# EmbersArc/SCpp

Hardware: AMD Instinct MI355X
Metric: converged SCvx trajectories/sec (RocketQuat, K=50) at 1/2/4/8 MI355X (higher is better)
Workload: dtype f64

## Files before the change

scpp_amd/csrc/discretize_kernel.h:

```cpp
#pragma once
#include "common.h"
#include <utility>

namespace scpp
{

template <class F, int... S>
__device__ inline void forEachStageImpl(F &&f, std::integer_sequence<int, S...>)
{
    (f(std::integral_constant<int, S>{}), ...);
}
template <class F>
__device__ inline void forEachStage(F &&f)
{
    forEachStageImpl(f, std::make_integer_sequence<int, RK_S>{});
}

#ifndef DISC_STEPS
#define DISC_STEPS 0
#endif
#ifndef DISC_MAX_STEP
#define DISC_MAX_STEP (12. / (14. * 5.))
#endif
constexpr int DISC_STEPS_MAX = 5;
#ifndef DISC_WAVES_PER_SIMD
#define DISC_WAVES_PER_SIMD 2
#endif

#ifndef DISC_STAGE_SCHEDULE
#define DISC_STAGE_SCHEDULE 1
#endif
#ifdef DISC_AD_JACOBIAN
#undef DISC_STAGE_SCHEDULE
#define DISC_STAGE_SCHEDULE 0
#endif
#ifndef DISC_LDS_GROUPS
#define DISC_LDS_GROUPS 1
#endif
#if defined(SCPP_HIP_EMU) || !DISC_LDS_GROUPS
#define DISC_READS_ISSUED()
#else
#define DISC_READS_ISSUED() __builtin_amdgcn_sched_barrier(0)
#endif
constexpr int rkNextStage(int s, bool skip)
{
    for (int r = s + 1; r < RK_S; r++)
        if (!skip || rkStageLive(r))
            return r;
    return RK_S;
}

template <class Model, bool FOH, bool VT>
struct DiscLayout
{
    static constexpr int NX = Model::NX, NU = Model::NU, NP = Model::NP;
    static constexpr int NJ = NX + NU;
    static constexpr int NCOLS = 1 + NX + NU + (FOH ? NU : 0) + (VT ? 1 : 0);
    static constexpr int NENT = NX * NCOLS;
    static constexpr int NG = WAVE / 16;
    static constexpr int EPL = (NCOLS + NG - 1) / NG;
    static constexpr int COL_S = 1, COL_PHI = 1 + (VT ? 1 : 0), COL_B = COL_PHI + NX, COL_C = COL_B + NU;
    static constexpr int NJP = (NJ + 1) & ~1;
};

template <class Model, bool FOH, bool VT>
struct DiscLds
{
    using L = DiscLayout<Model, FOH, VT>;
    __attribute__((aligned(16))) double Ys[32 * L::NX + 2];
#if DISC_STAGE_SCHEDULE
    __attribute__((aligned(16))) double Ys1[32 * L::NX + 2];
#endif
#ifdef DISC_AD_JACOBIAN
    __attribute__((aligned(16))) double Jm[L::NX * L::NJP];
    double fv[L::NX];
    double cst[L::NP + 2 * L::NU + 1];
#else
    double uh[DISC_STEPS_MAX * RK_S * (Model::JacobianRows::NUAUX + 1 + L::NU)];
    __attribute__((aligned(16))) double Wt[Model::JacobianTable::NW];
    double cst[L::NP + 2 * L::NU + Model::JacobianRows::NAUX + 1];
#endif
};

template <class Model, bool FOH, bool VT, bool SKIP = (RK_SKIP_DEAD != 0)>
__device__ __forceinline__ void discretizeSegment(int B, int K, const double *__restrict__ X, const double *__restrict__ U,
                                                  const double *__restrict__ sigma, const double *__restrict__ par, int par_stride,
                                                  const int *__restrict__ active, double *__restrict__ Aout, double *__restrict__ Bout,
                                                  double *__restrict__ Cout, double *__restrict__ Sout, double *__restrict__ Zout, int steps_opt,
                                                  const long inst, const int k, DiscLds<Model, FOH, VT> *lds)
{
    using L = DiscLayout<Model, FOH, VT>;
    constexpr int NX = L::NX, NU = L::NU, NP = L::NP, NJ = L::NJ, NJP = L::NJP, NCOLS = L::NCOLS, NG = L::NG, EPL = L::EPL;

    static_assert(NX <= 16 && NCOLS + NG <= 32 && NG == 4, "one 16-row tile of states, two 16-column tiles of V");
    auto &Ys = lds->Ys;
#ifndef DISC_AD_JACOBIAN
    constexpr int NAUX = Model::JacobianRows::NAUX;
    constexpr int NUAUX = Model::JacobianRows::NUAUX;
    constexpr int UHP = NUAUX + 1 + NU;
    auto &uh = lds->uh;
#define DISC_TABLE_ROWS 1
    using TB = typename Model::JacobianTable;
    auto &Wt = lds->Wt;
#else
    constexpr int NAUX = 0;
    auto &Jm = lds->Jm;
    auto &fv = lds->fv;
#endif
    auto &cst = lds->cst;

    const int lane = threadIdx.x;
    for (int i = lane; i < 32 * NX + 2; i += WAVE)
        Ys[i] = 0.;
    const int nseg = K - 1;
    if (inst >= B)
        return;
    if (active && active[inst] == 0)
        return;

    const double sg = sigma[inst];
    const double dt = VT ? 1. / double(K - 1) : sg / double(K - 1);
    const double tscale = VT ? sg : 1.;
    int nsteps = DISC_STEPS > 0 ? DISC_STEPS : steps_opt;
    if (nsteps <= 0)
    {
        const double seg_seconds = fabs(sg) / double(K - 1);
        nsteps = int(ceil(seg_seconds / DISC_MAX_STEP));
        nsteps = nsteps < 1 ? 1 : (nsteps > DISC_STEPS_MAX ? DISC_STEPS_MAX : nsteps);
    }
    nsteps = uniformInt(nsteps);
    double p[NP];
#pragma unroll
    for (int i = 0; i < NP; i++)
        p[i] = par[inst * par_stride + i];
    double u0[NU], u1[NU];
#pragma unroll
    for (int i = 0; i < NU; i++)
    {
        u0[i] = U[(inst * K + k) * NU + i];
        u1[i] = FOH ? U[(inst * K + k + 1) * NU + i] : u0[i];
    }

    if (lane == 0)
    {
#pragma unroll
        for (int i = 0; i < NP; i++)
            cst[i] = p[i];
#pragma unroll
        for (int i = 0; i < NU; i++)
        {
            cst[NP + i] = u0[i];
            cst[NP + NU + i] = u1[i];
        }
#ifndef DISC_AD_JACOBIAN
        double aux0[NAUX];
        Model::JacobianRows::prepare(p, aux0);
#pragma unroll
        for (int i = 0; i < NAUX; i++)
            cst[NP + 2 * NU + i] = aux0[i];
#endif
    }
#ifndef DISC_AD_JACOBIAN
    {
        const double hh = dt / double(nsteps);
        for (int e = lane; e < nsteps * RK_S; e += WAVE)
        {
            const double tse = double(e / RK_S) * hh + RK_C[e % RK_S] * hh;
            const double fre = FOH ? tse / dt : 0.;
            double ue[NU], ua[NUAUX];
#pragma unroll
            for (int i = 0; i < NU; i++)
                ue[i] = u0[i] + fre * (u1[i] - u0[i]);
            Model::JacobianRows::prepareInput(ue, p, ua);
#pragma unroll
            for (int i = 0; i < NUAUX; i++)
                uh[e * UHP + i] = ua[i];
            uh[e * UHP + NUAUX] = fre;
#pragma unroll
            for (int i = 0; i < NU; i++)
                uh[e * UHP + NUAUX + 1 + i] = ue[i];
        }
    }
#endif
#ifdef DISC_TABLE_ROWS
    for (int i = lane; i < TB::NW; i += WAVE)
        Wt[i] = (i == TB::W_ONE) ? 1. : 0.;
#endif
    WAVE_SYNC();
#ifdef DISC_TABLE_ROWS
    if (lane == 0)
    {
#pragma unroll
        for (int i = 0; i < NP; i++)
            Wt[TB::W_PAR + i] = p[i];
#pragma unroll
        for (int i = 0; i < NAUX; i++)
            Wt[TB::W_AUX + i] = cst[NP + 2 * NU + i];
    }
    double tcf[2][TB::MAXMON];
    unsigned tof[2][TB::MAXMON][2];
    int ttg[2];
#pragma unroll
    for (int ps = 0; ps < 2; ps++)
    {
        const int slot = ps * 64 + lane;
        ttg[ps] = TB::target(slot);
#pragma unroll
        for (int q = 0; q < TB::MAXMON; q++)
        {
            tcf[ps][q] = TB::coef(slot, q);
            tof[ps][q][0] = unsigned(TB::factor(slot, q, 0) * 8) | (unsigned(TB::factor(slot, q, 1) * 8) << 16);
            tof[ps][q][1] = unsigned(TB::factor(slot, q, 2) * 8) | (unsigned(TB::factor(slot, q, 3) * 8) << 16);
        }
    }
    WAVE_SYNC();
#endif
    const int row = lane & 15, g = lane >> 4;
    const bool lane_on = row < NX;
#ifndef SCPP_HIP_EMU
    __builtin_assume(g >= 0 && g < NG);
#endif
    const double x0r = lane_on ? X[(inst * K + k) * NX + row] : 0.;
    double y[EPL];
    bool eon[EPL];
#pragma unroll
    for (int m = 0; m < EPL; m++)
    {
        const int c = m * NG + g;
        eon[m] = lane_on && c < NCOLS;
        double v = 0.;
        if (c == 0)
            v = x0r;
        else if (c >= L::COL_PHI && c < L::COL_PHI + NX)
            v = (c - L::COL_PHI == row) ? 1. : 0.;
        y[m] = eon[m] ? v : 0.;
    }

    double kk[RK_S][EPL];
    const double h = dt / double(nsteps);
#ifdef DISC_PROFILE
    long long tA = 0, tB = 0, tC = 0;
    const long long tk0 = clock64();
#endif

    for (int step = 0; step < nsteps; step++)
    {
        const double t0 = double(step) * h;
        forEachStage([&](auto sc) {
            constexpr int s = decltype(sc)::value;
            if (SKIP && !rkStageLive(s))
                return;
#ifdef DISC_PROFILE
            const long long p0 = clock64();
#endif
            const double ts = t0 + RK_C[s] * h;
#pragma unroll
            for (int m = 0; m < EPL; m++)
            {
                double acc = 0.;
#pragma unroll
                for (int j = 0; j < s; j++)
                    if (RK_A[s][j] != 0.)
                        acc += RK_A[s][j] * kk[j][m];
                const double ys = y[m] + h * acc;
                if (eon[m])
                    Ys[(m * NG + g) * NX + row] = ys;
#ifdef DISC_TABLE_ROWS
                if (m == 0 && g == 0 && lane_on)
                    Wt[TB::W_X + row] = ys;
#endif
            }
            WAVE_SYNC();
#ifdef DISC_PROFILE
            const long long p1 = clock64();
            tA += p1 - p0;
#endif
#ifndef DISC_AD_JACOBIAN
            const double frac = FOH ? uh[(step * RK_S + s) * UHP + NUAUX] : 0.;
#else
            const double frac = FOH ? ts / dt : 0.;
#endif
            double jr[NJ];
            double fr;
#ifdef DISC_TABLE_ROWS
            double bsel[4];
            {
                const int e = step * RK_S + s;
                if (lane < NU)
                    Wt[TB::W_U + lane] = uh[e * UHP + NUAUX + 1 + lane];
                else if (lane < NU + NUAUX)
                    Wt[TB::W_UAUX + lane - NU] = uh[e * UHP + lane - NU];
                {
                    double hh[TB::NH];
                    TB::evalHoists(Ys, uh + e * UHP + NUAUX + 1, cst, cst + NP + 2 * NU, uh + e * UHP, hh);
                    if (lane == 0)
                    {
#pragma unroll
                        for (int i = 0; i < TB::NH; i++)
                            Wt[TB::W_H + i] = hh[i];
                    }
                }
                WAVE_SYNC();
                const char *wb = reinterpret_cast<const char *>(Wt);
#pragma unroll
                for (int ps = 0; ps < 2; ps++)
                {
                    double val = 0.;
#pragma unroll
                    for (int q = 0; q < (ps == 0 ? TB::MAXMON : TB::MAXMON_B); q++)
                    {
                        const double f0 = *reinterpret_cast<const double *>(wb + (tof[ps][q][0] & 0xFFFFu));
                        const double f1 = *reinterpret_cast<const double *>(wb + (tof[ps][q][0] >> 16));
                        const double f2 = *reinterpret_cast<const double *>(wb + (tof[ps][q][1] & 0xFFFFu));
                        const double f3 = *reinterpret_cast<const double *>(wb + (tof[ps][q][1] >> 16));
                        val += ((tcf[ps][q] * f0) * f1) * (f2 * f3);
                    }
                    if (ttg[ps] >= 0)
                        Wt[ttg[ps]] = val;
                    WAVE_SYNC();
                }
                const int rowc = lane_on ? row : 0;
#pragma unroll
                for (int t = 0; t < 4; t++)
                {
                    const double v = Wt[TB::W_J + rowc * NJ + (4 * t + g < NX ? 4 * t + g : 0)];
                    bsel[t] = (4 * t + g < NX) ? v : 0.;
                }
                fr = Wt[TB::W_F + rowc];
            }
#elif !defined(DISC_AD_JACOBIAN)
            {
                int zo = 0;
#ifndef SCPP_HIP_EMU
                asm volatile("" : "+v"(zo));
#endif
                const double *cv = cst + zo;
                double pl[NP], xs[NX], us[NU], ax[NAUX], ux[NUAUX];
#pragma unroll
                for (int i = 0; i < NUAUX; i++)
                    ux[i] = uh[(step * RK_S + s) * UHP + i];
#pragma unroll
                for (int i = 0; i < NP; i++)
                    pl[i] = cv[i];
#pragma unroll
                for (int i = 0; i < NAUX; i++)
                    ax[i] = cv[NP + 2 * NU + i];
#pragma unroll
                for (int i = 0; i < NX; i++)
                    xs[i] = Ys[i];
#pragma unroll
                for (int i = 0; i < NU; i++)
                {
                    const double a0 = cv[NP + i], a1 = cv[NP + NU + i];
                    us[i] = a0 + frac * (a1 - a0);
                }
                fr = Model::JacobianRows::row(row, xs, us, pl, ax, ux, jr);
            }
#else
            if (lane < NJ)
            {
                Dual1 xd[NX], ud[NU], fd[NX];
                int zo = 0;
#ifndef SCPP_HIP_EMU
                asm volatile("" : "+v"(zo));
#endif
                const double *cv = cst + zo;
                double pl[NP];
#pragma unroll
                for (int i = 0; i < NP; i++)
                    pl[i] = cv[i];
#pragma unroll
                for (int i = 0; i < NX; i++)
                    xd[i] = Dual1(Ys[i], (lane == i) ? 1. : 0.);
#pragma unroll
                for (int i = 0; i < NU; i++)
                {
                    const double a0 = cv[NP + i], a1 = cv[NP + NU + i];
                    ud[i] = Dual1(a0 + frac * (a1 - a0), (lane == NX + i) ? 1. : 0.);
                }
                Model::template systemFlowMap<Dual1>(xd, ud, pl, fd);
#pragma unroll
                for (int i = 0; i < NX; i++)
                    Jm[i * NJP + lane] = tscale * fd[i].d;
                if (lane == 0)
                {
#pragma unroll
                    for (int i = 0; i < NX; i++)
                        fv[i] = fd[i].v;
                }
            }
            WAVE_SYNC();
#pragma unroll
            for (int j = 0; j < NJ; j++)
                jr[j] = Jm[row * NJP + j];
            fr = fv[row];
#endif
#ifdef DISC_PROFILE
            const long long p2 = clock64();
            tB += p2 - p1;
#endif
            {
                const double alphaB = FOH ? (1. - frac) : 1.;
                d4_t acc0 = {0., 0., 0., 0.}, acc1 = {0., 0., 0., 0.};
#pragma unroll
                for (int t = 0; t < 4; t++)
                {
                    const int kx = g + 4 * t;
#ifdef DISC_TABLE_ROWS
                    double b = bsel[t];
#else
                    double b = (4 * t < NX) ? jr[4 * t < NX ? 4 * t : 0] : 0.;
#pragma unroll
                    for (int q = 1; q < 4; q++)
                        b = (g == q) ? ((4 * t + q < NX) ? jr[4 * t + q < NX ? 4 * t + q : 0] : 0.) : b;
#endif
#ifndef DISC_AD_JACOBIAN
                    b *= tscale;
#endif
                    acc0 = __builtin_amdgcn_mfma_f64_16x16x4f64(Ys[row * NX + kx], b, acc0, 0, 0, 0);
                    if (NCOLS > 16)
                        acc1 = __builtin_amdgcn_mfma_f64_16x16x4f64(Ys[(16 + row) * NX + kx], b, acc1, 0, 0, 0);
                }
#pragma unroll
                for (int m = 0; m < EPL; m++)
                {
                    const int c = m * NG + g;
                    const double acc = m < 4 ? acc0[m < 4 ? m : 0] : acc1[m >= 4 ? m - 4 : 0];
                    double d = acc;
                    const bool slotB = m * NG < L::COL_B + NU && m * NG + NG > L::COL_B;
                    const bool slotC = FOH && m * NG < L::COL_C + NU && m * NG + NG > L::COL_C;
                    if (slotB || slotC)
                    {
                        const bool isB = c >= L::COL_B && c < L::COL_B + NU;
                        const bool isC = FOH && c >= L::COL_C && c < L::COL_C + NU;
                        const int jj = isB ? c - L::COL_B : isC ? c - L::COL_C : 0;
                        const double w = isB ? alphaB : isC ? frac : 0.;
#ifdef DISC_TABLE_ROWS
                        const double jb = Wt[TB::W_J + (lane_on ? row : 0) * NJ + NX + jj];
#else
                        double jb = jr[NX];
#pragma unroll
                        for (int q = 1; q < NU; q++)
                            jb = (jj == q) ? jr[NX + q] : jb;
#endif
#ifndef DISC_AD_JACOBIAN
                        d += (w * tscale) * jb;
#else
                        d += w * jb;
#endif
                    }
                    if (VT && m * NG <= L::COL_S && m * NG + NG > L::COL_S)
                        d = (c == L::COL_S) ? d + fr : d;
                    if (m == 0)
                        d = (c == 0) ? tscale * fr : d;
                    kk[s][m] = d;
                }
            }
            WAVE_SYNC();
#ifdef DISC_PROFILE
            tC += clock64() - p2;
#endif
        });
#pragma unroll
        for (int m = 0; m < EPL; m++)
        {
            double acc = 0.;
#pragma unroll
            for (int s = 0; s < RK_S; s++)
                if (RK_B[s] != 0.)
                    acc += RK_B[s] * kk[s][m];
            y[m] += h * acc;
        }
    }

#ifdef DISC_PROFILE
    if (blockIdx.x == 4096 && lane == 0)
        printf("disc profile (cycles/segment): stage-value %lld  AD %lld  product %lld  total %lld\n", tA, tB, tC, (long long)(clock64() - tk0));
#endif
    const long seg = inst * nseg + k;
#pragma unroll
    for (int m = 0; m < EPL; m++)
    {
        const int c = m * NG + g;
        if (!eon[m])
            continue;
        Ys[c * NX + row] = y[m];
        if (c >= L::COL_PHI && c < L::COL_PHI + NX)
            Aout[seg * NX * NX + row * NX + (c - L::COL_PHI)] = y[m];
        else if (c >= L::COL_B && c < L::COL_B + NU)
            Bout[seg * NX * NU + row * NU + (c - L::COL_B)] = y[m];
        else if (FOH && c >= L::COL_C && c < L::COL_C + NU)
            Cout[seg * NX * NU + row * NU + (c - L::COL_C)] = y[m];
        else if (VT && c == L::COL_S)
            Sout[seg * NX + row] = y[m];
    }
    if (lane < NX)
        Ys[NCOLS * NX + lane] = x0r;
    WAVE_SYNC();
    if (lane < NX)
    {
        double z = Ys[lane];
#pragma unroll
        for (int j = 0; j < NX; j++)
            z -= Ys[(L::COL_PHI + j) * NX + lane] * Ys[NCOLS * NX + j];
#pragma unroll
        for (int j = 0; j < NU; j++)
        {
            z -= Ys[(L::COL_B + j) * NX + lane] * u0[j];
            if (FOH)
                z -= Ys[(L::COL_C + j) * NX + lane] * u1[j];
        }
        if (VT)
            z -= Ys[L::COL_S * NX + lane] * sg;
        Zout[seg * NX + lane] = z;
    }
}

#if DISC_STAGE_SCHEDULE
template <class Model>
struct DiscTableSlots
{
    using TB = typename Model::JacobianTable;
    double tcf[2][TB::MAXMON];
    unsigned tof[2][TB::MAXMON][2];
    int ttg[2];
};

template <class Model, bool FOH, bool VT>
__device__ __forceinline__ bool discretizeSetup(int B, const double *__restrict__ par, int par_stride, const int *__restrict__ active, const long inst,
                                                DiscLds<Model, FOH, VT> *lds, DiscTableSlots<Model> &ts)
{
    using L = DiscLayout<Model, FOH, VT>;
    using TB = typename Model::JacobianTable;
    constexpr int NX = L::NX, NU = L::NU, NP = L::NP, NAUX = Model::JacobianRows::NAUX;
    static_assert(NX <= 16 && L::NCOLS + L::NG <= 32 && L::NG == 4, "one 16-row tile of states, two 16-column tiles of V");
    const int lane = threadIdx.x;
    if (inst >= B)
        return false;
    if (active && active[inst] == 0)
        return false;
    for (int i = lane; i < 32 * NX + 2; i += WAVE)
    {
        lds->Ys[i] = 0.;
        lds->Ys1[i] = 0.;
    }
    for (int i = lane; i < TB::NW; i += WAVE)
        lds->Wt[i] = (i == TB::W_ONE) ? 1. : 0.;
    WAVE_SYNC();
    if (lane == 0)
    {
        double p[NP], aux0[NAUX];
#pragma unroll
        for (int i = 0; i < NP; i++)
            p[i] = par[inst * par_stride + i];
        Model::JacobianRows::prepare(p, aux0);
#pragma unroll
        for (int i = 0; i < NP; i++)
        {
            lds->cst[i] = p[i];
            lds->Wt[TB::W_PAR + i] = p[i];
        }
#pragma unroll
        for (int i = 0; i < NAUX; i++)
        {
            lds->cst[NP + 2 * NU + i] = aux0[i];
            lds->Wt[TB::W_AUX + i] = aux0[i];
        }
    }
#pragma unroll
    for (int ps = 0; ps < 2; ps++)
    {
        const int slot = ps * 64 + lane;
        ts.ttg[ps] = TB::target(slot);
#pragma unroll
        for (int q = 0; q < TB::MAXMON; q++)
        {
            ts.tcf[ps][q] = TB::coef(slot, q);
            ts.tof[ps][q][0] = unsigned(TB::factor(slot, q, 0) * 8) | (unsigned(TB::factor(slot, q, 1) * 8) << 16);
            ts.tof[ps][q][1] = unsigned(TB::factor(slot, q, 2) * 8) | (unsigned(TB::factor(slot, q, 3) * 8) << 16);
        }
    }
    WAVE_SYNC();
    return true;
}

template <class Model, bool FOH, bool VT, bool SKIP>
__device__ __forceinline__ void discretizeSegmentBody(int K, const double *__restrict__ X, const double *__restrict__ U, const double *__restrict__ sigma,
                                                      double *__restrict__ Aout, double *__restrict__ Bout, double *__restrict__ Cout,
                                                      double *__restrict__ Sout, double *__restrict__ Zout, int steps_opt, const long inst, const int k,
                                                      DiscLds<Model, FOH, VT> *lds, const DiscTableSlots<Model> &ts)
{
    using L = DiscLayout<Model, FOH, VT>;
    using TB = typename Model::JacobianTable;
    constexpr int NX = L::NX, NU = L::NU, NP = L::NP, NJ = L::NJ, NCOLS = L::NCOLS, NG = L::NG, EPL = L::EPL;
    constexpr int NAUX = Model::JacobianRows::NAUX, NUAUX = Model::JacobianRows::NUAUX, UHP = NUAUX + 1 + NU;
    constexpr int NLIVE = SKIP ? rkLiveBefore(RK_S) : RK_S;
    auto &Ys = lds->Ys;
    auto &uh = lds->uh;
    auto &Wt = lds->Wt;
    auto &cst = lds->cst;
    (void)NAUX;

    const int lane = threadIdx.x;
    const int nseg = K - 1;
    const double sg = sigma[inst];
    const double dt = VT ? 1. / double(K - 1) : sg / double(K - 1);
    const double tscale = VT ? sg : 1.;
    int nsteps = DISC_STEPS > 0 ? DISC_STEPS : steps_opt;
    if (nsteps <= 0)
    {
        const double seg_seconds = fabs(sg) / double(K - 1);
        nsteps = int(ceil(seg_seconds / DISC_MAX_STEP));
        nsteps = nsteps < 1 ? 1 : (nsteps > DISC_STEPS_MAX ? DISC_STEPS_MAX : nsteps);
    }
    nsteps = uniformInt(nsteps);
    const int row = lane & 15, g = lane >> 4;
    const bool lane_on = row < NX;
#ifndef SCPP_HIP_EMU
    __builtin_assume(g >= 0 && g < NG);
#endif
    double u0[NU], u1[NU];
#pragma unroll
    for (int i = 0; i < NU; i++)
    {
        u0[i] = U[(inst * K + k) * NU + i];
        u1[i] = FOH ? U[(inst * K + k + 1) * NU + i] : u0[i];
    }
#if DISC_LDS_GROUPS
    const double x0r = lane_on ? X[(inst * K + k) * NX + row] : 0.;
    DISC_READS_ISSUED();
#endif
    if (lane == 0)
    {
#pragma unroll
        for (int i = 0; i < NU; i++)
        {
            cst[NP + i] = u0[i];
            cst[NP + NU + i] = u1[i];
        }
    }
    {
        double p[NP];
#pragma unroll
        for (int i = 0; i < NP; i++)
            p[i] = cst[i];
        const double hh = dt / double(nsteps);
        for (int e = lane; e < nsteps * RK_S; e += WAVE)
        {
            const double tse = double(e / RK_S) * hh + RK_C[e % RK_S] * hh;
            const double fre = FOH ? tse / dt : 0.;
            double ue[NU], ua[NUAUX];
#pragma unroll
            for (int i = 0; i < NU; i++)
                ue[i] = u0[i] + fre * (u1[i] - u0[i]);
            Model::JacobianRows::prepareInput(ue, p, ua);
#pragma unroll
            for (int i = 0; i < NUAUX; i++)
                uh[e * UHP + i] = ua[i];
            uh[e * UHP + NUAUX] = fre;
#pragma unroll
            for (int i = 0; i < NU; i++)
                uh[e * UHP + NUAUX + 1 + i] = ue[i];
        }
    }
    WAVE_SYNC();

#if !DISC_LDS_GROUPS
    const double x0r = lane_on ? X[(inst * K + k) * NX + row] : 0.;
#endif
    double y[EPL];
    bool eon[EPL];
#pragma unroll
    for (int m = 0; m < EPL; m++)
    {
        const int c = m * NG + g;
        eon[m] = lane_on && c < NCOLS;
        double v = 0.;
        if (c == 0)
            v = x0r;
        else if (c >= L::COL_PHI && c < L::COL_PHI + NX)
            v = (c - L::COL_PHI == row) ? 1. : 0.;
        y[m] = eon[m] ? v : 0.;
    }

    double kk[RK_S][EPL];
    const double h = dt / double(nsteps);
#if DISC_LDS_GROUPS
    const bool ucp = lane < NU + NUAUX;
    const int usrc = lane < NU ? NUAUX + 1 + lane : (ucp ? lane - NU : 0);
    const int udst = lane < NU ? TB::W_U + lane : TB::W_UAUX + lane - NU;
    double uop_n = uh[usrc];
    double frac_n = FOH ? uh[NUAUX] : 0.;
#endif
    for (int step = 0; step < nsteps; step++)
    {
        forEachStage([&](auto sc) {
            constexpr int s = decltype(sc)::value;
            if (SKIP && !rkStageLive(s))
                return;
            constexpr int ord = SKIP ? rkLiveBefore(s) : s;
            const int buf = (NLIVE % 2 == 0) ? (ord & 1) : ((ord + step) & 1);
            double *Yb = buf ? lds->Ys1 : lds->Ys;
            const int e = step * RK_S + s;
            double ys0 = 0.;
#pragma unroll
            for (int m = 0; m < EPL; m++)
            {
                double acc = 0.;
#pragma unroll
                for (int j = 0; j < s; j++)
                    if (RK_A[s][j] != 0.)
                        acc += RK_A[s][j] * kk[j][m];
                const double ys = y[m] + h * acc;
                if (eon[m])
                    Yb[(m * NG + g) * NX + row] = ys;
                if (m == 0)
                {
                    ys0 = ys;
                    if (g == 0 && lane_on)
                        Wt[TB::W_X + row] = ys;
                }
            }
            {
                double xs[NX], hh[TB::NH];
#pragma unroll
                for (int i = 0; i < NX; i++)
                    xs[i] = readLane(ys0, i);
                TB::evalHoists(xs, uh + e * UHP + NUAUX + 1, cst, cst + NP + 2 * NU, uh + e * UHP, hh);
                if (lane == 0)
                {
#pragma unroll
                    for (int i = 0; i < TB::NH; i++)
                        Wt[TB::W_H + i] = hh[i];
                }
#if DISC_LDS_GROUPS
                if (ucp)
                    Wt[udst] = uop_n;
#else
                if (lane < NU)
                    Wt[TB::W_U + lane] = uh[e * UHP + NUAUX + 1 + lane];
                else if (lane < NU + NUAUX)
                    Wt[TB::W_UAUX + lane - NU] = uh[e * UHP + lane - NU];
#endif
            }
            WAVE_SYNC();
#if DISC_LDS_GROUPS
            const double frac = frac_n;
#else
            const double frac = FOH ? uh[e * UHP + NUAUX] : 0.;
#endif
            const char *wb = reinterpret_cast<const char *>(Wt);
#pragma unroll
            for (int ps = 0; ps < 2; ps++)
            {
                double val = 0.;
#if DISC_LDS_GROUPS
                double fc[TB::MAXMON][4];
#pragma unroll
                for (int q = 0; q < (ps == 0 ? TB::MAXMON : TB::MAXMON_B); q++)
                {
                    fc[q][0] = *reinterpret_cast<const double *>(wb + (ts.tof[ps][q][0] & 0xFFFFu));
                    fc[q][1] = *reinterpret_cast<const double *>(wb + (ts.tof[ps][q][0] >> 16));
                    fc[q][2] = *reinterpret_cast<const double *>(wb + (ts.tof[ps][q][1] & 0xFFFFu));
                    fc[q][3] = *reinterpret_cast<const double *>(wb + (ts.tof[ps][q][1] >> 16));
                }
                DISC_READS_ISSUED();
#pragma unroll
                for (int q = 0; q < (ps == 0 ? TB::MAXMON : TB::MAXMON_B); q++)
                    val += ((ts.tcf[ps][q] * fc[q][0]) * fc[q][1]) * (fc[q][2] * fc[q][3]);
#else
#pragma unroll
                for (int q = 0; q < (ps == 0 ? TB::MAXMON : TB::MAXMON_B); q++)
                {
                    const double f0 = *reinterpret_cast<const double *>(wb + (ts.tof[ps][q][0] & 0xFFFFu));
                    const double f1 = *reinterpret_cast<const double *>(wb + (ts.tof[ps][q][0] >> 16));
                    const double f2 = *reinterpret_cast<const double *>(wb + (ts.tof[ps][q][1] & 0xFFFFu));
                    const double f3 = *reinterpret_cast<const double *>(wb + (ts.tof[ps][q][1] >> 16));
                    val += ((ts.tcf[ps][q] * f0) * f1) * (f2 * f3);
                }
#endif
                if (ts.ttg[ps] >= 0)
                    Wt[ts.ttg[ps]] = val;
                WAVE_SYNC();
            }
            const int rowc = lane_on ? row : 0;
            double bsel[4];
#pragma unroll
            for (int t = 0; t < 4; t++)
            {
                const double v = Wt[TB::W_J + rowc * NJ + (4 * t + g < NX ? 4 * t + g : 0)];
#if DISC_LDS_GROUPS
                bsel[t] = v;
#else
                bsel[t] = (4 * t + g < NX) ? v : 0.;
#endif
            }
            const double fr = Wt[TB::W_F + rowc];
#if DISC_LDS_GROUPS
            auto forcingCol = [&](int m) {
                const int c = m * NG + g;
                const bool slotB = m * NG < L::COL_B + NU && m * NG + NG > L::COL_B;
                const bool slotC = FOH && m * NG < L::COL_C + NU && m * NG + NG > L::COL_C;
                if (!(slotB || slotC))
                    return -1;
                const bool isB = c >= L::COL_B && c < L::COL_B + NU;
                const bool isC = FOH && c >= L::COL_C && c < L::COL_C + NU;
                return isB ? c - L::COL_B : isC ? c - L::COL_C : 0;
            };
            double jbv[EPL], ya0[4], ya1[4];
#pragma unroll
            for (int m = 0; m < EPL; m++)
            {
                const int jj = forcingCol(m);
                jbv[m] = jj >= 0 ? Wt[TB::W_J + rowc * NJ + NX + jj] : 0.;
            }
#pragma unroll
            for (int t = 0; t < 4; t++)
            {
                ya0[t] = Yb[row * NX + g + 4 * t];
                ya1[t] = NCOLS > 16 ? Yb[(16 + row) * NX + g + 4 * t] : 0.;
            }
            {
                constexpr int sn = rkNextStage(s, SKIP);
                const int en = sn < RK_S ? step * RK_S + sn : (step + 1 < nsteps ? (step + 1) * RK_S : 0);
                uop_n = uh[en * UHP + usrc];
                frac_n = FOH ? uh[en * UHP + NUAUX] : 0.;
            }
            DISC_READS_ISSUED();
#pragma unroll
            for (int t = 0; t < 4; t++)
                bsel[t] = (4 * t + g < NX) ? bsel[t] : 0.;
#endif
            const double alphaB = FOH ? (1. - frac) : 1.;
            d4_t acc0 = {0., 0., 0., 0.}, acc1 = {0., 0., 0., 0.};
#pragma unroll
            for (int t = 0; t < 4; t++)
            {
                const int kx = g + 4 * t;
                const double b = bsel[t] * tscale;
#if DISC_LDS_GROUPS
                (void)kx;
                acc0 = __builtin_amdgcn_mfma_f64_16x16x4f64(ya0[t], b, acc0, 0, 0, 0);
                if (NCOLS > 16)
                    acc1 = __builtin_amdgcn_mfma_f64_16x16x4f64(ya1[t], b, acc1, 0, 0, 0);
#else
                acc0 = __builtin_amdgcn_mfma_f64_16x16x4f64(Yb[row * NX + kx], b, acc0, 0, 0, 0);
                if (NCOLS > 16)
                    acc1 = __builtin_amdgcn_mfma_f64_16x16x4f64(Yb[(16 + row) * NX + kx], b, acc1, 0, 0, 0);
#endif
            }
#pragma unroll
            for (int m = 0; m < EPL; m++)
            {
                const int c = m * NG + g;
                const double acc = m < 4 ? acc0[m < 4 ? m : 0] : acc1[m >= 4 ? m - 4 : 0];
                double d = acc;
                const bool slotB = m * NG < L::COL_B + NU && m * NG + NG > L::COL_B;
                const bool slotC = FOH && m * NG < L::COL_C + NU && m * NG + NG > L::COL_C;
                if (slotB || slotC)
                {
                    const bool isB = c >= L::COL_B && c < L::COL_B + NU;
                    const bool isC = FOH && c >= L::COL_C && c < L::COL_C + NU;
                    const int jj = isB ? c - L::COL_B : isC ? c - L::COL_C : 0;
                    const double w = isB ? alphaB : isC ? frac : 0.;
#if DISC_LDS_GROUPS
                    (void)jj;
                    const double jb = jbv[m];
#else
                    const double jb = Wt[TB::W_J + rowc * NJ + NX + jj];
#endif
                    d += (w * tscale) * jb;
                }
                if (VT && m * NG <= L::COL_S && m * NG + NG > L::COL_S)
                    d = (c == L::COL_S) ? d + fr : d;
                if (m == 0)
                    d = (c == 0) ? tscale * fr : d;
                kk[s][m] = d;
            }
        });
#pragma unroll
        for (int m = 0; m < EPL; m++)
        {
            double acc = 0.;
#pragma unroll
            for (int s = 0; s < RK_S; s++)
                if (RK_B[s] != 0.)
                    acc += RK_B[s] * kk[s][m];
            y[m] += h * acc;
        }
    }
    WAVE_SYNC();

    const long seg = inst * nseg + k;
#pragma unroll
    for (int m = 0; m < EPL; m++)
    {
        const int c = m * NG + g;
        if (!eon[m])
            continue;
        Ys[c * NX + row] = y[m];
        if (c >= L::COL_PHI && c < L::COL_PHI + NX)
            Aout[seg * NX * NX + row * NX + (c - L::COL_PHI)] = y[m];
        else if (c >= L::COL_B && c < L::COL_B + NU)
            Bout[seg * NX * NU + row * NU + (c - L::COL_B)] = y[m];
        else if (FOH && c >= L::COL_C && c < L::COL_C + NU)
            Cout[seg * NX * NU + row * NU + (c - L::COL_C)] = y[m];
        else if (VT && c == L::COL_S)
            Sout[seg * NX + row] = y[m];
    }
    if (lane < NX)
        Ys[NCOLS * NX + lane] = x0r;
    WAVE_SYNC();
    if (lane < NX)
    {
#if DISC_LDS_GROUPS
        double za[NX], zx[NX], zb[NU], zc[NU];
        double z = Ys[lane];
#pragma unroll
        for (int j = 0; j < NX; j++)
        {
            za[j] = Ys[(L::COL_PHI + j) * NX + lane];
            zx[j] = Ys[NCOLS * NX + j];
        }
#pragma unroll
        for (int j = 0; j < NU; j++)
        {
            zb[j] = Ys[(L::COL_B + j) * NX + lane];
            zc[j] = FOH ? Ys[(L::COL_C + j) * NX + lane] : 0.;
        }
        const double zs = VT ? Ys[L::COL_S * NX + lane] : 0.;
        DISC_READS_ISSUED();
#pragma unroll
        for (int j = 0; j < NX; j++)
            z -= za[j] * zx[j];
#pragma unroll
        for (int j = 0; j < NU; j++)
        {
            z -= zb[j] * u0[j];
            if (FOH)
                z -= zc[j] * u1[j];
        }
        if (VT)
            z -= zs * sg;
#else
        double z = Ys[lane];
#pragma unroll
        for (int j = 0; j < NX; j++)
            z -= Ys[(L::COL_PHI + j) * NX + lane] * Ys[NCOLS * NX + j];
#pragma unroll
        for (int j = 0; j < NU; j++)
        {
            z -= Ys[(L::COL_B + j) * NX + lane] * u0[j];
            if (FOH)
                z -= Ys[(L::COL_C + j) * NX + lane] * u1[j];
        }
        if (VT)
            z -= Ys[L::COL_S * NX + lane] * sg;
#endif
        Zout[seg * NX + lane] = z;
    }
    WAVE_SYNC();
    if (lane < NX)
        Ys[NCOLS * NX + lane] = 0.;
    WAVE_SYNC();
}
#endif

template <class Model, bool FOH, bool VT, int SCHED = DISC_STAGE_SCHEDULE, bool SKIP = (RK_SKIP_DEAD != 0)>
__device__ __forceinline__ void discretizeSegments(int B, int K, const double *__restrict__ X, const double *__restrict__ U,
                                                   const double *__restrict__ sigma, const double *__restrict__ par, int par_stride,
                                                   const int *__restrict__ active, double *__restrict__ Aout, double *__restrict__ Bout,
                                                   double *__restrict__ Cout, double *__restrict__ Sout, double *__restrict__ Zout, int steps_opt,
                                                   const long inst, const int k0, const int k1, DiscLds<Model, FOH, VT> *lds)
{
#if DISC_STAGE_SCHEDULE
    if constexpr (SCHED != 0)
    {
        DiscTableSlots<Model> ts;
        if (!discretizeSetup<Model, FOH, VT>(B, par, par_stride, active, inst, lds, ts))
            return;
        for (int k = k0; k < k1; k++)
            discretizeSegmentBody<Model, FOH, VT, SKIP>(K, X, U, sigma, Aout, Bout, Cout, Sout, Zout, steps_opt, inst, k, lds, ts);
    }
    else
#endif
    {
        for (int k = k0; k < k1; k++)
        {
            discretizeSegment<Model, FOH, VT, SKIP>(B, K, X, U, sigma, par, par_stride, active, Aout, Bout, Cout, Sout, Zout, steps_opt, inst, k, lds);
            WAVE_SYNC();
        }
    }
}

template <class Model, bool FOH, bool VT, int SCHED = DISC_STAGE_SCHEDULE, bool SKIP = (RK_SKIP_DEAD != 0)>
__global__ void __launch_bounds__(WAVE, DISC_WAVES_PER_SIMD)
    discretize_kernel(int B, int K, const double *__restrict__ X, const double *__restrict__ U,
                      const double *__restrict__ sigma, const double *__restrict__ par, int par_stride,
                      const int *__restrict__ active,
                      double *__restrict__ Aout, double *__restrict__ Bout, double *__restrict__ Cout,
                      double *__restrict__ Sout, double *__restrict__ Zout, int steps_opt)
{
    const int nseg = K - 1;
    const long b = blockIdx.x;
    const long xcd = b & 7, gb = b >> 3;
    const long inst = (gb / nseg) * 8 + xcd;
    const int k = int(gb % nseg);
    __shared__ DiscLds<Model, FOH, VT> lds;
    discretizeSegments<Model, FOH, VT, SCHED, SKIP>(B, K, X, U, sigma, par, par_stride, active, Aout, Bout, Cout, Sout, Zout, steps_opt, inst, k, k + 1, &lds);
}

template <class Model>
__global__ void simulate_kernel(int B, const double *__restrict__ par, int par_stride, const double *__restrict__ dtv,
                                const double *__restrict__ u0v, const double *__restrict__ u1v, double *__restrict__ x,
                                const int *__restrict__ active)
{
    constexpr int NX = Model::NX, NU = Model::NU, NP = Model::NP;
    const long i = long(blockIdx.x) * blockDim.x + threadIdx.x;
    if (i >= B)
        return;
    if (active && active[i] == 0)
        return;
    double p[NP], u0[NU], u1[NU], y[NX], kk[RK_S][NX];
    for (int j = 0; j < NP; j++)
        p[j] = par[i * par_stride + j];
    for (int j = 0; j < NU; j++)
    {
        u0[j] = u0v[i * NU + j];
        u1[j] = u1v[i * NU + j];
    }
    for (int j = 0; j < NX; j++)
        y[j] = x[i * NX + j];
    const double dt = dtv[i];
    const double h = dt / 20.;
    for (int step = 0; step < 20; step++)
    {
        const double t0 = double(step) * h;
#pragma unroll
        for (int s = 0; s < RK_S; s++)
        {
            if (RK_SKIP_DEAD && !rkStageLive(s))
                continue;
            double ys[NX], u[NU];
            const double ts = t0 + RK_C[s] * h;
            for (int j = 0; j < NX; j++)
            {
                double acc = 0.;
#pragma unroll
                for (int q = 0; q < s; q++)
                    if (RK_A[s][q] != 0.)
                        acc += RK_A[s][q] * kk[q][j];
                ys[j] = y[j] + h * acc;
            }
            for (int j = 0; j < NU; j++)
                u[j] = u0[j] + ts / dt * (u1[j] - u0[j]);
            Model::template systemFlowMap<double>(ys, u, p, kk[s]);
        }
        for (int j = 0; j < NX; j++)
        {
            double acc = 0.;
#pragma unroll
            for (int s = 0; s < RK_S; s++)
                if (RK_B[s] != 0.)
                    acc += RK_B[s] * kk[s][j];
            y[j] += h * acc;
        }
    }
    for (int j = 0; j < NX; j++)
        x[i * NX + j] = y[j];
}

}
```

Measured before the change: 6506.

## Sink predicated LDS stores to dummy slots and precompute RK stage prefix sums

Replaces lane-predicated LDS stores (Ys, Wt state, hoists, u operands, table targets) with unconditional stores that inactive lanes send to padding sink slots appended to the LDS arrays. This removes exec-mask branching around stores. Separately, it accumulates the Runge-Kutta A-row (or B-row) partial sum over the already-known stages while the MFMAs for the current stage are in flight. The next stage then only adds the newest k term, taking that arithmetic off the critical path. The cost is extra LDS footprint and some register pressure from the pre[] and ydst[] arrays.

```diff
diff --git a/scpp_amd/csrc/discretize_kernel.h b/scpp_amd/csrc/discretize_kernel.h
--- a/scpp_amd/csrc/discretize_kernel.h
+++ b/scpp_amd/csrc/discretize_kernel.h
@@ -42,12 +42,25 @@
 #else
 #define DISC_READS_ISSUED() __builtin_amdgcn_sched_barrier(0)
 #endif
+#ifndef DISC_SINK_STORES
+#define DISC_SINK_STORES 1
+#endif
+#ifndef DISC_RK_PREFIX
+#define DISC_RK_PREFIX 1
+#endif
 constexpr int rkNextStage(int s, bool skip)
 {
     for (int r = s + 1; r < RK_S; r++)
         if (!skip || rkStageLive(r))
             return r;
     return RK_S;
+}
+constexpr int rkPrevStage(int s, bool skip)
+{
+    for (int r = s - 1; r >= 0; r--)
+        if (!skip || rkStageLive(r))
+            return r;
+    return -1;
 }
 
 template <class Model, bool FOH, bool VT>
@@ -61,15 +74,17 @@
     static constexpr int EPL = (NCOLS + NG - 1) / NG;
     static constexpr int COL_S = 1, COL_PHI = 1 + (VT ? 1 : 0), COL_B = COL_PHI + NX, COL_C = COL_B + NU;
     static constexpr int NJP = (NJ + 1) & ~1;
+    static constexpr int YS_N = 32 * NX + 2;
+    static constexpr int SINK = (DISC_STAGE_SCHEDULE && DISC_SINK_STORES) ? WAVE : 0;
 };
 
 template <class Model, bool FOH, bool VT>
 struct DiscLds
 {
     using L = DiscLayout<Model, FOH, VT>;
-    __attribute__((aligned(16))) double Ys[32 * L::NX + 2];
+    __attribute__((aligned(16))) double Ys[L::YS_N + L::SINK];
 #if DISC_STAGE_SCHEDULE
-    __attribute__((aligned(16))) double Ys1[32 * L::NX + 2];
+    __attribute__((aligned(16))) double Ys1[L::YS_N + L::SINK];
 #endif
 #ifdef DISC_AD_JACOBIAN
     __attribute__((aligned(16))) double Jm[L::NX * L::NJP];
@@ -77,7 +92,7 @@
     double cst[L::NP + 2 * L::NU + 1];
 #else
     double uh[DISC_STEPS_MAX * RK_S * (Model::JacobianRows::NUAUX + 1 + L::NU)];
-    __attribute__((aligned(16))) double Wt[Model::JacobianTable::NW];
+    __attribute__((aligned(16))) double Wt[Model::JacobianTable::NW + (L::SINK ? L::SINK + Model::JacobianTable::NH : 0)];
     double cst[L::NP + 2 * L::NU + Model::JacobianRows::NAUX + 1];
 #endif
 };
@@ -572,6 +587,10 @@
     {
         const int slot = ps * 64 + lane;
         ts.ttg[ps] = TB::target(slot);
+#if DISC_SINK_STORES
+        if (ts.ttg[ps] < 0)
+            ts.ttg[ps] = TB::NW + lane;
+#endif
 #pragma unroll
         for (int q = 0; q < TB::MAXMON; q++)
         {
@@ -688,10 +707,25 @@
 #if DISC_LDS_GROUPS
     const bool ucp = lane < NU + NUAUX;
     const int usrc = lane < NU ? NUAUX + 1 + lane : (ucp ? lane - NU : 0);
+#if DISC_SINK_STORES
+    const int udst = lane < NU ? TB::W_U + lane : (ucp ? TB::W_UAUX + lane - NU : TB::NW + lane);
+#else
     const int udst = lane < NU ? TB::W_U + lane : TB::W_UAUX + lane - NU;
+#endif
     double uop_n = uh[usrc];
     double frac_n = FOH ? uh[NUAUX] : 0.;
 #endif
+#if DISC_SINK_STORES
+    constexpr int MFULL = NCOLS / NG;
+    int ydst[EPL];
+#pragma unroll
+    for (int m = 0; m < EPL; m++)
+        ydst[m] = eon[m] ? (m * NG + g) * NX + row : L::YS_N + lane;
+    const int wxdst = (g == 0 && lane_on) ? TB::W_X + row : TB::NW + lane;
+    const int whdst = lane == 0 ? TB::W_H : TB::NW + lane;
+#endif
+    double pre[EPL] = {};
+    (void)pre;
     for (int step = 0; step < nsteps; step++)
     {
         forEachStage([&](auto sc) {
@@ -703,15 +737,24 @@
             double *Yb = buf ? lds->Ys1 : lds->Ys;
             const int e = step * RK_S + s;
             double ys0 = 0.;
+            constexpr int sp = DISC_RK_PREFIX ? rkPrevStage(s, SKIP) : -1;
+#if DISC_SINK_STORES
+            double ysv[EPL];
+#endif
 #pragma unroll
             for (int m = 0; m < EPL; m++)
             {
-                double acc = 0.;
-#pragma unroll
-                for (int j = 0; j < s; j++)
+                double acc = sp >= 0 ? pre[m] : 0.;
+#pragma unroll
+                for (int j = (sp >= 0 ? sp : 0); j < s; j++)
                     if (RK_A[s][j] != 0.)
                         acc += RK_A[s][j] * kk[j][m];
                 const double ys = y[m] + h * acc;
+#if DISC_SINK_STORES
+                ysv[m] = ys;
+                if (m == 0)
+                    ys0 = ys;
+#else
                 if (eon[m])
                     Yb[(m * NG + g) * NX + row] = ys;
                 if (m == 0)
@@ -720,20 +763,41 @@
                     if (g == 0 && lane_on)
                         Wt[TB::W_X + row] = ys;
                 }
-            }
+#endif
+            }
+#if DISC_SINK_STORES
+            if (lane_on)
+            {
+#pragma unroll
+                for (int m = 0; m < MFULL; m++)
+                    Yb[(m * NG + g) * NX + row] = ysv[m];
+            }
+#pragma unroll
+            for (int m = MFULL; m < EPL; m++)
+                Yb[ydst[m]] = ysv[m];
+            Wt[wxdst] = ys0;
+#endif
             {
                 double xs[NX], hh[TB::NH];
 #pragma unroll
                 for (int i = 0; i < NX; i++)
                     xs[i] = readLane(ys0, i);
                 TB::evalHoists(xs, uh + e * UHP + NUAUX + 1, cst, cst + NP + 2 * NU, uh + e * UHP, hh);
+#if DISC_SINK_STORES
+#pragma unroll
+                for (int i = 0; i < TB::NH; i++)
+                    Wt[whdst + i] = hh[i];
+#else
                 if (lane == 0)
                 {
 #pragma unroll
                     for (int i = 0; i < TB::NH; i++)
                         Wt[TB::W_H + i] = hh[i];
                 }
-#if DISC_LDS_GROUPS
+#endif
+#if DISC_LDS_GROUPS && DISC_SINK_STORES
+                Wt[udst] = uop_n;
+#elif DISC_LDS_GROUPS
                 if (ucp)
                     Wt[udst] = uop_n;
 #else
@@ -779,8 +843,12 @@
                     val += ((ts.tcf[ps][q] * f0) * f1) * (f2 * f3);
                 }
 #endif
+#if DISC_SINK_STORES
+                Wt[ts.ttg[ps]] = val;
+#else
                 if (ts.ttg[ps] >= 0)
                     Wt[ts.ttg[ps]] = val;
+#endif
                 WAVE_SYNC();
             }
             const int rowc = lane_on ? row : 0;
@@ -849,6 +917,31 @@
                     acc1 = __builtin_amdgcn_mfma_f64_16x16x4f64(Yb[(16 + row) * NX + kx], b, acc1, 0, 0, 0);
 #endif
             }
+#if DISC_RK_PREFIX
+            {
+                constexpr int sn = rkNextStage(s, SKIP);
+#pragma unroll
+                for (int m = 0; m < EPL; m++)
+                {
+                    double acc = 0.;
+                    if constexpr (sn < RK_S)
+                    {
+#pragma unroll
+                        for (int j = 0; j < s; j++)
+                            if (RK_A[sn][j] != 0.)
+                                acc += RK_A[sn][j] * kk[j][m];
+                    }
+                    else
+                    {
+#pragma unroll
+                        for (int j = 0; j < s; j++)
+                            if (RK_B[j] != 0.)
+                                acc += RK_B[j] * kk[j][m];
+                    }
+                    pre[m] = acc;
+                }
+            }
+#endif
 #pragma unroll
             for (int m = 0; m < EPL; m++)
             {
@@ -878,12 +971,13 @@
                 kk[s][m] = d;
             }
         });
+        constexpr int SLAST = DISC_RK_PREFIX ? rkPrevStage(RK_S, SKIP) : 0;
 #pragma unroll
         for (int m = 0; m < EPL; m++)
         {
-            double acc = 0.;
-#pragma unroll
-            for (int s = 0; s < RK_S; s++)
+            double acc = DISC_RK_PREFIX ? pre[m] : 0.;
+#pragma unroll
+            for (int s = SLAST; s < RK_S; s++)
                 if (RK_B[s] != 0.)
                     acc += RK_B[s] * kk[s][m];
             y[m] += h * acc;
```

New measurement: 6554, median of 6. No clear change (+0.7%).
